# mjb3/DiscretePOMP.jl

Measured on NVIDIA B200. Metric: particle-obs steps/sec (bootstrap PF), higher is better.
Workload: dtype f32 event loop + f64 weights/scan (int32 state)

## Files before the change

### discretepomp.jl_b200/csrc/dpomp_dev.cuh

```cuda
#pragma once
#include <cuda_runtime.h>
#include <stdint.h>
#include <stdio.h>

#include "../../include/dpomp.h"

namespace dpomp {

#ifndef DPOMP_BLOCK_THREADS
#define DPOMP_BLOCK_THREADS 128
#endif
#ifndef DPOMP_ITEMS_LARGE
#define DPOMP_ITEMS_LARGE 8
#endif
#ifndef DPOMP_ITEMS_SMALL
#define DPOMP_ITEMS_SMALL 2
#endif
#ifdef DPOMP_PHASE_TIMERS
#ifndef DPOMP_PHASE_OBS
#define DPOMP_PHASE_OBS 50
#endif
static __device__ unsigned long long g_dpomp_phase[2][4096][8];
__device__ __forceinline__ unsigned long long dpomp_gtime() {
    unsigned long long t;
    asm volatile("mov.u64 %0, %%globaltimer;" : "=l"(t));
    return t;
}
#define DPOMP_STAMP(K, P)                                                                                   \
    do {                                                                                                    \
        if (threadIdx.x == 0 && a.t == DPOMP_PHASE_OBS && blockIdx.x < 4096) g_dpomp_phase[K][blockIdx.x][P] = dpomp_gtime(); \
    } while (0)
#define DPOMP_STAMP_NEXT(K, P)                                                                              \
    do {                                                                                                    \
        if (threadIdx.x == 0 && a.t == DPOMP_PHASE_OBS + 1 && blockIdx.x < 4096) g_dpomp_phase[K][blockIdx.x][P] = dpomp_gtime(); \
    } while (0)
#else
#define DPOMP_STAMP(K, P) do { } while (0)
#define DPOMP_STAMP_NEXT(K, P) do { } while (0)
#endif
#ifdef DPOMP_BOUNDS_CHECK
#define DPOMP_CHECK_IDX(i, n)                                                                                          \
    do {                                                                                                               \
        if (!((long long)(i) >= 0 && (long long)(i) < (long long)(n))) {                                               \
            printf("dpomp bounds: %s:%d: index %lld outside [0, %lld)\n", __FILE__, __LINE__, (long long)(i), (long long)(n)); \
            __trap();                                                                                                  \
        }                                                                                                              \
    } while (0)
#else
#define DPOMP_CHECK_IDX(i, n) do { } while (0)
#endif
constexpr int kBlockThreads = DPOMP_BLOCK_THREADS;
constexpr int kItemsLarge = DPOMP_ITEMS_LARGE, kItemsSmall = DPOMP_ITEMS_SMALL;

__device__ __forceinline__ void pdl_wait() {
#if __CUDA_ARCH__ >= 900
    cudaGridDependencySynchronize();
#endif
}
__device__ __forceinline__ void pdl_trigger() {
#if __CUDA_ARCH__ >= 900 && defined(DPOMP_PDL_TRIGGER)
    cudaTriggerProgrammaticLaunchCompletion();
#endif
}
template <typename... KArgs, typename... Args>
inline cudaError_t launch_pdl(void (*kern)(KArgs...), unsigned grid, unsigned block, size_t smem, cudaStream_t stream, Args... args) {
    cudaLaunchConfig_t cfg{};
    cfg.gridDim = dim3(grid);
    cfg.blockDim = dim3(block);
    cfg.dynamicSmemBytes = smem;
    cfg.stream = stream;
    cudaLaunchAttribute attr[1];
    attr[0].id = cudaLaunchAttributeProgrammaticStreamSerialization;
    attr[0].val.programmaticStreamSerializationAllowed = 1;
    cfg.attrs = attr;
    cfg.numAttrs = 1;
    return cudaLaunchKernelEx(&cfg, kern, args...);
}
constexpr int kGroupTiles = 32;
constexpr int kDeferGroups = 64;
__device__ __forceinline__ double tile_cw(double grp_off, double grp_f, double tile_o, double tile_f, double incl) {
    return __dadd_rn(grp_off, __dmul_rn(grp_f, __dadd_rn(tile_o, __dmul_rn(tile_f, incl))));
}
struct Level2 {
    double big_m, big_s;
};
template <bool CG = true>
__device__ __forceinline__ Level2 combine_level2(const double* gm_b, const double* gs_b, int ngroups, double* grp_f_out,
                                                 double* grp_off_out) {
    auto ld = [](const double* p) -> double {
        if constexpr (CG) return __ldcg(p); else return *p;
    };
    const int lane = threadIdx.x & 31;
    double big_m = -INFINITY;
    for (int i = lane; i < ngroups; i += 32) big_m = fmax(big_m, ld(gm_b + i));
#pragma unroll
    for (int d = 16; d > 0; d >>= 1) big_m = fmax(big_m, __shfl_xor_sync(0xffffffffu, big_m, d));
    double carry = 0.0;
    for (int c0 = 0; c0 < ngroups; c0 += 32) {
        const int i = c0 + lane;
        const bool have = i < ngroups;
        const double mg = have ? ld(gm_b + i) : -INFINITY;
        const double f = (mg == -INFINITY) ? 0.0 : exp(mg - big_m);
        double inc = have ? __dmul_rn(f, ld(gs_b + i)) : 0.0;
#pragma unroll
        for (int d = 1; d < 32; d <<= 1) {
            const double y = __shfl_up_sync(0xffffffffu, inc, d);
            if (lane >= d) inc = __dadd_rn(y, inc);
        }
        double prev = __shfl_up_sync(0xffffffffu, inc, 1);
        if (lane == 0) prev = 0.0;
        if (have) {
            grp_f_out[i] = f;
            grp_off_out[i] = __dadd_rn(carry, prev);
        }
        carry = __dadd_rn(carry, __shfl_sync(0xffffffffu, inc, 31));
    }
    return Level2{big_m, carry};
}
struct ChunkPerm {
    int ncf, m, q, r;
};
__host__ __device__ __forceinline__ int chunk_sigma(const ChunkPerm& p, int rr, int qq) {
    return rr * p.q + (rr < p.r ? rr : p.r) + qq;
}
__host__ __device__ __forceinline__ long long perm_pos(const ChunkPerm& p, long long i) {
    const int k = (int)(i >> 5);
    if (k >= p.ncf) return i;
    return ((long long)chunk_sigma(p, k % p.m, k / p.m) << 5) | (i & 31);
}
inline ChunkPerm make_chunk_perm(int scatter_mode, long long n, int ntiles) {
    ChunkPerm p{0, 1, 0, 0};
    if (scatter_mode != 0 && ntiles > 1) {
        p.ncf = (int)(n >> 5);
        p.m = ntiles;
        p.q = p.ncf / ntiles;
        p.r = p.ncf % ntiles;
    }
    return p;
}

constexpr uint32_t kTagSim = 0u;
constexpr uint32_t kTagResample = 1u;

struct Philox4 {
    uint32_t w0, w1, w2, w3;
};

__device__ __forceinline__ Philox4 philox4x32_10(uint32_t c0, uint32_t c1, uint32_t c2, uint32_t c3, uint32_t k0,
                                                 uint32_t k1) {
#pragma unroll
    for (int r = 0; r < 10; ++r) {
        const uint32_t hi0 = __umulhi(0xD2511F53u, c0), lo0 = 0xD2511F53u * c0;
        const uint32_t hi1 = __umulhi(0xCD9E8D57u, c2), lo1 = 0xCD9E8D57u * c2;
        const uint32_t n0 = hi1 ^ c1 ^ k0, n2 = hi0 ^ c3 ^ k1;
        c0 = n0; c1 = lo1; c2 = n2; c3 = lo0;
        k0 += 0x9E3779B9u; k1 += 0xBB67AE85u;
    }
    return Philox4{c0, c1, c2, c3};
}

__device__ __forceinline__ Philox4 stream_draw(uint64_t key, uint32_t particle, uint32_t filter, uint32_t obs,
                                               uint32_t tag, uint32_t block) {
    return philox4x32_10(particle, filter, obs, (tag << 30) | block, (uint32_t)key, (uint32_t)(key >> 32));
}

__device__ __forceinline__ uint2 philox2x32_10(uint32_t c0, uint32_t c1, uint32_t key) {
#pragma unroll
    for (int r = 0; r < 10; ++r) {
        const uint32_t hi = __umulhi(0xD256D193u, c0), lo = 0xD256D193u * c0;
        c0 = hi ^ key ^ c1;
        c1 = lo;
        key += 0x9E3779B9u;
    }
    return make_uint2(c0, c1);
}

struct SimStream {
    uint32_t k, a, b;
};
__device__ __forceinline__ SimStream sim_stream_init(uint64_t key, uint32_t filter, uint32_t obs) {
    const Philox4 p = stream_draw(key, 0u, filter, obs, kTagSim, 0u);
    return SimStream{p.w0, p.w1, p.w2};
}

__device__ __forceinline__ double u32_open_f64(uint32_t w) { return ((double)w + 0.5) * 0x1.0p-32; }
__device__ __forceinline__ float u32_wait_f32(uint32_t w) { return fmaf(__uint2float_rn(w), 0x1.0p-32f, 0x1.0p-33f); }
__device__ __forceinline__ float u32_event_f32(uint32_t w) { return __uint2float_rz(w) * 0x1.0p-32f; }
__device__ __forceinline__ double u53(uint32_t hi, uint32_t lo) {
    return (double)(((uint64_t)hi << 21) | (uint64_t)(lo >> 11)) * 0x1.0p-53;
}

template <int ITEMS, bool TAIL_SYNC = true>
__device__ __forceinline__ double tile_scan(const double (&a)[ITEMS], double (&incl)[ITEMS], double (&excl)[ITEMS],
                                            double* warp_tot) {
    const int lane = threadIdx.x & 31, warp = threadIdx.x >> 5;
    double r[ITEMS];
    r[0] = a[0];
#pragma unroll
    for (int k = 1; k < ITEMS; ++k) r[k] = __dadd_rn(r[k - 1], a[k]);
    double inc = r[ITEMS - 1];
#pragma unroll
    for (int d = 1; d < 32; d <<= 1) {
        const double y = __shfl_up_sync(0xffffffffu, inc, d);
        if (lane >= d) inc = __dadd_rn(y, inc);
    }
    double prev = __shfl_up_sync(0xffffffffu, inc, 1);
    if (lane == 0) prev = 0.0;
    if (lane == 31) warp_tot[warp] = inc;
    __syncthreads();
    double prefix = 0.0, total = 0.0;
#pragma unroll
    for (int w = 0; w < kBlockThreads / 32; ++w) {
        if (w == warp) prefix = total;
        total = __dadd_rn(total, warp_tot[w]);
    }
    const double base = __dadd_rn(prefix, prev);
#pragma unroll
    for (int k = 0; k < ITEMS; ++k) {
        incl[k] = __dadd_rn(base, r[k]);
        excl[k] = __dadd_rn(base, k > 0 ? r[k - 1] : 0.0);
    }
    if constexpr (TAIL_SYNC) __syncthreads();
    return total;
}

__device__ __forceinline__ double block_max(double v, double* warp_scratch) {
    const int lane = threadIdx.x & 31, warp = threadIdx.x >> 5;
#pragma unroll
    for (int d = 16; d > 0; d >>= 1) v = fmax(v, __shfl_xor_sync(0xffffffffu, v, d));
    if (lane == 0) warp_scratch[warp] = v;
    __syncthreads();
    double m = warp_scratch[0];
#pragma unroll
    for (int w = 1; w < kBlockThreads / 32; ++w) m = fmax(m, warp_scratch[w]);
    __syncthreads();
    return m;
}

struct ResampleCtx {
    int rs_type;
    long long n;
    double dn;
    double inv_n;
    bool pow2;
    double s;
    double inv_s;
    double r1_over_n;
    uint64_t key;
    uint32_t filter, obs;
};

__device__ __forceinline__ double div_by_n(const ResampleCtx& c, double v) {
    return c.pow2 ? v * c.inv_n : __ddiv_rn(v, c.dn);
}

template <int RS = 0>
__device__ __forceinline__ double resample_u(const ResampleCtx& c, int i ) {
    const double q = div_by_n(c, (double)(i - 1));
    double r = c.r1_over_n;
    if ((RS ? RS : c.rs_type) == DPOMP_RS_STRATIFIED) {
        const Philox4 p = stream_draw(c.key, (uint32_t)(i - 1), c.filter, c.obs, kTagResample, 1u);
        r = div_by_n(c, u53(p.w0, p.w1));
    }
    return __dmul_rn(__dadd_rn(r, q), c.s);
}

template <int RS = 0>
__device__ __forceinline__ int resample_ecount_guess(const ResampleCtx& c, double v, bool& exact) {
    const int n = (int)c.n;
    exact = true;
    if (!(c.s > 0.0)) return n;
    double g;
    if ((RS ? RS : c.rs_type) == DPOMP_RS_STRATIFIED) {
        g = floor(v * c.inv_s * c.dn);
    } else {
        const double t = (v * c.inv_s - c.r1_over_n) * c.dn;
        const double fl = floor(t);
        const double frac = t - fl;
#ifndef DPOMP_NO_ECOUNT_FAST
        if (frac > 0x1.0p-12 && frac < 1.0 - 0x1.0p-12 && t > 0.0 && t < c.dn - 1.0) return (int)fl + 1;
#endif
        g = fl + 1.0;
    }
    exact = false;
    return (int)fmin(fmax(g, 0.0), c.dn);
}
template <int RS = 0>
__device__ __forceinline__ int resample_ecount_correct(const ResampleCtx& c, double v, int e) {
    const int n = (int)c.n;
    while (e < n && resample_u<RS>(c, e + 1) <= v) ++e;
    while (e > 0 && resample_u<RS>(c, e) > v) --e;
    return e;
}
template <int RS = 0>
__device__ __forceinline__ long long resample_ecount(const ResampleCtx& c, double v) {
    bool exact;
    const int e = resample_ecount_guess<RS>(c, v, exact);
    return exact ? e : resample_ecount_correct<RS>(c, v, e);
}

__device__ __forceinline__ ResampleCtx make_resample_ctx(int rs_type, long long n, double s, uint64_t key,
                                                         uint32_t filter, uint32_t obs, double r_systematic) {
    ResampleCtx c;
    c.rs_type = rs_type;
    c.n = n;
    c.dn = (double)n;
    c.pow2 = (n & (n - 1)) == 0;
    c.inv_n = 1.0 / c.dn;
    c.s = s;
    c.inv_s = (s > 0.0) ? 1.0 / s : 0.0;
    c.key = key;
    c.filter = filter;
    c.obs = obs;
    c.r1_over_n = div_by_n(c, r_systematic);
    return c;
}

}
```

### discretepomp.jl_b200/csrc/pf_sim.cuh

```cuda
#pragma once
#include <type_traits>

#include "dpomp_dev.cuh"
#include "dpomp_internal.cuh"
#include "dpomp_models.cuh"
#include "obs_count.cuh"
#include "pf_resample.cuh"

namespace dpomp {

template <typename Real> struct Arith;
template <> struct Arith<float> {
    static __device__ __forceinline__ float mul(float a, float b) { return a * b; }
    static __device__ __forceinline__ float add(float a, float b) { return a + b; }
    static __device__ __forceinline__ float div(float a, float b) { return __fdividef(a, b); }
};
template <> struct Arith<double> {
    static __device__ __forceinline__ double mul(double a, double b) { return __dmul_rn(a, b); }
    static __device__ __forceinline__ double add(double a, double b) { return __dadd_rn(a, b); }
    static __device__ __forceinline__ double div(double a, double b) { return __ddiv_rn(a, b); }
};

#ifndef DPOMP_SIM_ILP
#define DPOMP_SIM_ILP 1
#endif
#ifndef DPOMP_SIM_PIPE
#define DPOMP_SIM_PIPE 1
#endif
#ifndef DPOMP_SIM_MINB
#define DPOMP_SIM_MINB (DPOMP_BLOCK_THREADS == 128 ? 7 : 4)
#endif
template <typename Real, int C, int E>
constexpr int sim_min_blocks() { return sizeof(Real) == 4 ? DPOMP_SIM_MINB : 1; }

template <int N>
struct alignas(4 * N) IntVec { int v[N]; };

template <typename Real, int C, int E, int MODEL>
__device__ __forceinline__ void cum_rates(const DevModel<Real, C, E>& m, const Real (&par)[E], const Real (&x)[C], Real (&cum)[E]) {
    if constexpr (MODEL != kModelGeneric) {
        using BM = Builtin<MODEL>;
#pragma unroll
        for (int e = 0; e < E; ++e) {
            Real rate = Arith<Real>::mul(par[e], x[BM::A(e)]);
            if (BM::B(e) >= 0) rate = Arith<Real>::mul(rate, x[BM::B(e) >= 0 ? BM::B(e) : 0]);
            cum[e] = (e == 0) ? rate : Arith<Real>::add(cum[e - 1], rate);
        }
    } else {
#pragma unroll
        for (int e = 0; e < E; ++e) {
            Real l1 = m.k1[e], l2 = m.k2[e];
#pragma unroll
            for (int c = 0; c < C; ++c) {
                l1 += m.f1[e][c] * x[c];
                l2 += m.f2[e][c] * x[c];
            }
            Real rate = Arith<Real>::mul(Arith<Real>::mul(par[e], l1), l2);
            if (m.any_den && m.has_den[e]) {
                Real dn = m.kd[e];
#pragma unroll
                for (int c = 0; c < C; ++c) dn += m.dn[e][c] * x[c];
                rate = (dn == (Real)0) ? (Real)0 : Arith<Real>::div(rate, dn);
            }
            cum[e] = (e == 0) ? rate : Arith<Real>::add(cum[e - 1], rate);
        }
    }
}

template <typename Real, int C, int E, int MODEL>
__device__ __forceinline__ void chosen_transition(const DevModel<Real, C, E>& m, const Real (&cum)[E], Real etc, Real (&dx)[C]) {
    if constexpr (MODEL != kModelGeneric) {
        using BM = Builtin<MODEL>;
#pragma unroll
        for (int c = 0; c < C; ++c) dx[c] = (Real)BM::T(E - 1, c);
#pragma unroll
        for (int i = E - 2; i >= 0; --i) {
            const bool hit = cum[i] > etc;
#pragma unroll
            for (int c = 0; c < C; ++c) dx[c] = hit ? (Real)BM::T(i, c) : dx[c];
        }
    } else {
#pragma unroll
        for (int c = 0; c < C; ++c) dx[c] = m.trans[E - 1][c];
#pragma unroll
        for (int i = E - 2; i >= 0; --i) {
            const bool hit = cum[i] > etc;
#pragma unroll
            for (int c = 0; c < C; ++c) dx[c] = hit ? m.trans[i][c] : dx[c];
        }
    }
}

constexpr int kModePlain = 0, kModeFused = 1, kModePersist = 2;
__device__ __forceinline__ unsigned int ld_acquire_u32(const unsigned int* p) {
    unsigned int v;
    asm volatile("ld.acquire.gpu.global.u32 %0, [%1];" : "=r"(v) : "l"(p) : "memory");
    return v;
}
constexpr int kModelCountObs = -1;
template <typename Real, int C, int E, int ITEMS, int MODEL = kModelGeneric, int MODE = kModePlain, int ILP = DPOMP_SIM_ILP>
__global__ void __launch_bounds__(kBlockThreads, sim_min_blocks<Real, C, E>())
pf_sim_weight_kernel(const __grid_constant__ DevModel<Real, C, E> m, const __grid_constant__ SimLaunch a) {
    constexpr bool COUNT = MODEL == kModelCountObs;
    constexpr int RMODEL = COUNT ? kModelGeneric : MODEL;
    constexpr int TILE = kBlockThreads * ITEMS;
    constexpr int CHUNK = 32 * ITEMS;
    constexpr bool kF32 = sizeof(Real) == 4;
    constexpr unsigned FULL = 0xffffffffu;
    constexpr bool FUSED = MODE == kModeFused, PERSIST = MODE == kModePersist;
    extern __shared__ __align__(16) unsigned char smem_raw[];
    using SState = typename std::conditional<kF32, float, int>::type;
    int* ovf_s = reinterpret_cast<int*>(smem_raw);
    SState* st_s = reinterpret_cast<SState*>(ovf_s + TILE);
    __shared__ double warp_scratch[kBlockThreads / 32];
    __shared__ unsigned warp_min_s[kBlockThreads / 32];
    __shared__ double wtab_s[kBlockThreads];
    __shared__ uint32_t stream_s[3];

    const int tid = threadIdx.x, lane = tid & 31, warp = tid >> 5;
    unsigned int logical = blockIdx.x;
    if constexpr (FUSED) {
        __shared__ unsigned int logical_s;
        if (a.work_counter) {
            if (tid == 0) logical_s = (unsigned int)(atomicAdd(a.work_counter, 1ull) - a.work_base);
            __syncthreads();
            logical = logical_s;
        }
    }
    const int tile = logical % a.ntiles;
    const int b = logical / a.ntiles;
    const long long base_n = (long long)tile * TILE;
    const uint32_t gfilter = a.filter_ids ? a.filter_ids[b] : a.filter0 + (uint32_t)b;
    const double* th = a.theta + (size_t)b * m.n_params;

    Real par[E];
#pragma unroll
    for (int e = 0; e < E; ++e) par[e] = m.par[e] >= 0 ? (Real)th[m.par[e]] : (Real)1;
    const uint32_t max_ev = (uint32_t)a.max_events;
    const int t_end = PERSIST ? a.t_last : a.t;
    int flip = 0;
    bool staged = false;
    bool wait_rows = false;
    __shared__ int warp_max_s[kBlockThreads / 32];
    __shared__ long long lohi_s[2];
    int t = a.t;
#pragma unroll 1
    do {
    const bool fresh = a.fresh && t == a.t;
    const int has_lik = PERSIST ? (a.obs_haslik[t] > 0) : a.has_lik;
    const bool do_rs = PERSIST ? (has_lik && t + 1 < a.n_obs_total) : (a.do_resample != 0);
    const bool resample_here = (FUSED || PERSIST) && do_rs;
    const double t_obs = a.obs_time[t];
    const double t_prev = fresh ? (m.t0_index > 0 ? th[m.t0_index - 1] : 0.0) : a.obs_time[t - 1];
    const double ysum = a.obs_ysum[t];
    int32_t* pop_b = ((PERSIST && (flip & 1)) ? a.pop_dst : a.pop) + (size_t)b * a.n_comp * a.n_pad;
    int32_t* pop_other = ((PERSIST && (flip & 1)) ? a.pop : a.pop_dst);
    const unsigned int gen_t = a.gen + (unsigned int)(t - a.t);

    DPOMP_STAMP(0, 0);
    DPOMP_STAMP_NEXT(0, 7);
    if (tid == 0) {
        const SimStream s0 = sim_stream_init(a.key, gfilter, (uint32_t)t);
        stream_s[0] = s0.k; stream_s[1] = s0.a; stream_s[2] = s0.b;
    }
    if constexpr (PERSIST) {
        if (wait_rows) {
            if (tid == 0) {
                const long long rem_rows = a.n - base_n;
                const unsigned int want = (unsigned int)(rem_rows < TILE ? (rem_rows > 0 ? rem_rows : 0) : TILE);
                unsigned int* cnt = a.rows_done + (size_t)b * a.ntiles + tile;
                while (ld_acquire_u32(cnt) < want) __nanosleep(40);
                *cnt = 0u;
            }
        }
        __syncthreads();
    } else {
        pdl_wait();
    }
    DPOMP_STAMP(0, 1);
    using Vec = IntVec<ITEMS>;
    {
        Vec z;
#pragma unroll
        for (int kk = 0; kk < ITEMS; ++kk) z.v[kk] = 0;
        *reinterpret_cast<Vec*>(ovf_s + tid * ITEMS) = z;
    }
    const int n_comp = (RMODEL != kModelGeneric) ? C : a.n_comp;
    if (PERSIST && staged) {
    } else if (!fresh) {
#pragma unroll
        for (int c = 0; c < C; ++c)
            if (c < n_comp)
            {
                DPOMP_CHECK_IDX(base_n + tid * ITEMS + ITEMS - 1, a.n_pad);
                const int32_t* src = pop_b + (size_t)c * a.n_pad + base_n + tid * ITEMS;
                Vec v;
                if constexpr (PERSIST) {
#pragma unroll
                    for (int kk = 0; kk < ITEMS; kk += (ITEMS % 4 == 0 ? 4 : 1)) {
                        if constexpr (ITEMS % 4 == 0) {
                            const int4 w4 = __ldcg(reinterpret_cast<const int4*>(src + kk));
                            v.v[kk] = w4.x; v.v[kk + 1] = w4.y; v.v[kk + 2] = w4.z; v.v[kk + 3] = w4.w;
                        } else {
                            v.v[kk] = __ldcg(src + kk);
                        }
                    }
                } else {
                    v = *reinterpret_cast<const Vec*>(src);
                }
#pragma unroll
                for (int kk = 0; kk < ITEMS; ++kk) st_s[c * TILE + tid * ITEMS + kk] = (SState)v.v[kk];
            }
    } else {
#pragma unroll
        for (int c = 0; c < C; ++c)
            if (c < n_comp) {
#pragma unroll
                for (int kk = 0; kk < ITEMS; ++kk) st_s[c * TILE + tid * ITEMS + kk] = (SState)m.ic[c];
            }
    }
    __syncthreads();
    DPOMP_STAMP(0, 2);
    const SimStream ss{stream_s[0], stream_s[1], stream_s[2]};

    constexpr int S = (kF32 && C <= 4 && E <= 3) ? ILP : 1;
    const int chunk0 = warp * CHUNK;
    const long long left = a.n - (base_n + chunk0);
    const int chunk_valid = left < CHUNK ? (left > 0 ? (int)left : 0) : CHUNK;
    const unsigned lt_mask = (1u << lane) - 1u;
    int next = 32 * S;
    int parked = 0;
    int q[S];
    bool active[S];
    Real x[S][C];
    Real tm[S];
    const Real tm0 = kF32 ? (Real)(t_obs - t_prev) : (Real)t_prev;
    uint32_t k[S];
    uint32_t pc[S];
    constexpr bool PIPE = DPOMP_SIM_PIPE && kF32 && S == 2;
    uint2 wn[S];
    unsigned long long ev_local = 0, ovf_local = 0;
#pragma unroll
    for (int s = 0; s < S; ++s) {
        const int slot = lane + 32 * s;
        active[s] = slot < chunk_valid;
        q[s] = chunk0 + (slot < CHUNK ? slot : lane);
        tm[s] = tm0;
        k[s] = 0;
        pc[s] = (uint32_t)(base_n + q[s]) ^ ss.a;
        if constexpr (PIPE) wn[s] = philox2x32_10(pc[s], 0u ^ ss.b, ss.k);
#pragma unroll
        for (int c = 0; c < C; ++c) x[s][c] = (c < n_comp) ? (Real)st_s[c * TILE + q[s]] : (Real)0;
    }

    while (parked < chunk_valid) {
        bool fin[S], ovf[S];
#pragma unroll
        for (int s = 0; s < S; ++s) {
            fin[s] = false;
            ovf[s] = false;
            if constexpr (kF32) {
                Real cum[E];
                cum_rates<Real, C, E, RMODEL>(m, par, x[s], cum);
                const Real rtot = cum[E - 1];
                uint2 w;
                if constexpr (PIPE) {
                    w = wn[s];
                    wn[s] = philox2x32_10(pc[s], (k[s] + 1u) ^ ss.b, ss.k);
                } else {
                    w = philox2x32_10(pc[s], k[s] ^ ss.b, ss.k);
                }
                const Real tmn = fmaf(__log2f(u32_wait_f32(w.x)), __fdividef(0.693147180559945f, rtot), tm[s]);
                const bool capped = k[s] >= max_ev;
                const bool go = (rtot > (Real)0) && !capped && (tmn >= (Real)0);
                Real dx[C];
                chosen_transition<Real, C, E, RMODEL>(m, cum, u32_event_f32(w.y) * rtot, dx);
                if (go) {
#pragma unroll
                    for (int c = 0; c < C; ++c) x[s][c] += dx[c];
                    ++k[s];
                    tm[s] = tmn;
                }
                fin[s] = active[s] && !go;
                ovf[s] = capped && (rtot > (Real)0);
            } else {
                if (active[s]) {
                    Real cum[E];
                    cum_rates<Real, C, E, RMODEL>(m, par, x[s], cum);
                    const Real rtot = cum[E - 1];
                    fin[s] = !(rtot > (Real)0);
                    if (!fin[s]) {
                        if (k[s] >= max_ev) {
                            fin[s] = true;
                            ovf[s] = true;
                        } else {
                            const uint2 w = philox2x32_10(pc[s], k[s] ^ ss.b, ss.k);
                            tm[s] = tm[s] - log(u32_open_f64(w.x)) / rtot;
                            fin[s] = tm[s] > t_obs;
                            if (!fin[s]) {
                                Real dx[C];
                                chosen_transition<Real, C, E, RMODEL>(m, cum, __dmul_rn(u32_open_f64(w.y), rtot), dx);
#pragma unroll
                                for (int c = 0; c < C; ++c) x[s][c] += dx[c];
                                ++k[s];
                            }
                        }
                    }
                }
            }
        }
#pragma unroll
        for (int s = 0; s < S; ++s) {
            const unsigned fmask = __ballot_sync(FULL, fin[s]);
            if (fmask) {
                if (fin[s]) {
                    DPOMP_CHECK_IDX(q[s], TILE);
#pragma unroll
                    for (int c = 0; c < C; ++c)
                        if (c < n_comp) st_s[c * TILE + q[s]] = (SState)x[s][c];
                    if (ovf[s]) {
                        ovf_s[q[s]] = 1;
                        ++ovf_local;
                    }
                    ev_local += k[s];
                    const int slot = next + __popc(fmask & lt_mask);
                    active[s] = slot < chunk_valid;
                    if (active[s]) {
                        q[s] = chunk0 + slot;
                        DPOMP_CHECK_IDX(q[s], TILE);
                        DPOMP_CHECK_IDX(slot, CHUNK);
                        DPOMP_CHECK_IDX(base_n + q[s], a.n);
                        pc[s] = (uint32_t)(base_n + q[s]) ^ ss.a;
#pragma unroll
                        for (int c = 0; c < C; ++c) x[s][c] = (c < n_comp) ? (Real)st_s[c * TILE + q[s]] : (Real)0;
                        tm[s] = tm0;
                        k[s] = 0;
                        if constexpr (PIPE) wn[s] = philox2x32_10(pc[s], 0u ^ ss.b, ss.k);
                    }
                }
                const int nf = __popc(fmask);
                next += nf;
                parked += nf;
            }
        }
    }
    __syncwarp();
    DPOMP_STAMP(0, 3);

    pdl_trigger();
    double av[ITEMS], incl[ITEMS], excl[ITEMS];
    auto logw_of = [&](double d) -> double {
        const double dd = __dmul_rn(d, d);
        const double quot = m.obs_tmp2_pow2 ? __dmul_rn(dd, m.obs_inv_tmp2) : __ddiv_rn(dd, m.obs_tmp2);
        return m.obs_tmp1 - quot;
    };
    constexpr unsigned kExcluded = 0xffffffffu;
    const bool int_obs = fabs(ysum) < 1073741824.0 && ysum == rint(ysum);
    double m_b;
    {
        int xs[ITEMS];
#pragma unroll
        for (int kk = 0; kk < ITEMS; ++kk) xs[kk] = 0;
#pragma unroll
        for (int c = 0; c < C; ++c)
            if (c < n_comp) {
                Vec v;
#pragma unroll
                for (int kk = 0; kk < ITEMS; ++kk) v.v[kk] = (int)st_s[c * TILE + tid * ITEMS + kk];
#pragma unroll
                for (int kk = 0; kk < ITEMS; ++kk) xs[kk] += m.xmask_i[c] * v.v[kk];
                if (!resample_here)
                    *reinterpret_cast<Vec*>(pop_b + (size_t)c * a.n_pad + base_n + tid * ITEMS) = v;
            }
        const Vec of = *reinterpret_cast<const Vec*>(ovf_s + tid * ITEMS);
        bool excluded[ITEMS];
#pragma unroll
        for (int kk = 0; kk < ITEMS; ++kk) excluded[kk] = !(base_n + tid * ITEMS + kk < a.n) || of.v[kk] != 0;

#pragma unroll
        for (int d = 16; d > 0; d >>= 1) {
            ev_local += __shfl_xor_sync(0xffffffffu, ev_local, d);
            ovf_local += __shfl_xor_sync(0xffffffffu, ovf_local, d);
        }
        if (lane == 1 && ev_local) atomicAdd(a.grp_ev + (size_t)b * a.ngroups + tile / kGroupTiles, ev_local);
        if (lane == 1 && ovf_local) atomicAdd(a.ovf_count, ovf_local);

        if constexpr (COUNT) {
            const CountObsConst cc = count_obs_const(a.cobs, th, t, ysum);
            double it[ITEMS], mloc = -INFINITY;
#pragma unroll
            for (int kk = 0; kk < ITEMS; ++kk) {
                it[kk] = excluded[kk] ? -INFINITY : count_obs_logpmf(cc, ysum, (double)xs[kk]);
                mloc = fmax(mloc, it[kk]);
            }
            if (a.record_logw) {
                double* lw_b = a.logw + (size_t)b * a.n_pad + base_n + (size_t)tid * ITEMS;
#pragma unroll
                for (int kk = 0; kk < ITEMS; ++kk) lw_b[kk] = it[kk];
            }
            m_b = block_max(mloc, warp_scratch);
            const double ref = (m_b == -INFINITY) ? 0.0 : m_b;
#pragma unroll
            for (int kk = 0; kk < ITEMS; ++kk) av[kk] = (it[kk] == -INFINITY) ? 0.0 : exp(it[kk] - ref);
        } else if (int_obs) {
            const int ys = (int)ysum;
            unsigned du[ITEMS], dloc = kExcluded;
#pragma unroll
            for (int kk = 0; kk < ITEMS; ++kk) {
                const long long df = (long long)ys - (long long)xs[kk];
                du[kk] = excluded[kk] ? kExcluded : (unsigned)(df < 0 ? -df : df);
                dloc = min(dloc, du[kk]);
            }
            dloc = __reduce_min_sync(0xffffffffu, dloc);
            if (lane == 0) warp_min_s[warp] = dloc;
            __syncthreads();
            unsigned dmin = warp_min_s[0];
#pragma unroll
            for (int w = 1; w < kBlockThreads / 32; ++w) dmin = min(dmin, warp_min_s[w]);
            if (dmin == kExcluded) {
                m_b = -INFINITY;
#pragma unroll
                for (int kk = 0; kk < ITEMS; ++kk) av[kk] = 0.0;
            } else {
                m_b = logw_of((double)dmin);
                wtab_s[tid] = exp(logw_of((double)dmin + (double)tid) - m_b);
                __syncthreads();
#pragma unroll
                for (int kk = 0; kk < ITEMS; ++kk) {
                    const unsigned off = du[kk] - dmin;
                    av[kk] = du[kk] == kExcluded ? 0.0
                           : (off < (unsigned)kBlockThreads ? wtab_s[off] : exp(logw_of((double)du[kk]) - m_b));
                    DPOMP_CHECK_IDX(du[kk] == kExcluded ? 0u : (off < (unsigned)kBlockThreads ? off : 0u), kBlockThreads);
                }
            }
            if (a.record_logw) {
                double* lw_b = a.logw + (size_t)b * a.n_pad + base_n + (size_t)tid * ITEMS;
#pragma unroll
                for (int kk = 0; kk < ITEMS; ++kk) lw_b[kk] = du[kk] == kExcluded ? -INFINITY : logw_of((double)du[kk]);
            }
        } else {
            double it[ITEMS], mloc = -INFINITY;
#pragma unroll
            for (int kk = 0; kk < ITEMS; ++kk) {
                it[kk] = excluded[kk] ? -INFINITY : logw_of(ysum - (double)xs[kk]);
                mloc = fmax(mloc, it[kk]);
            }
            if (a.record_logw) {
                double* lw_b = a.logw + (size_t)b * a.n_pad + base_n + (size_t)tid * ITEMS;
#pragma unroll
                for (int kk = 0; kk < ITEMS; ++kk) lw_b[kk] = it[kk];
            }
            m_b = block_max(mloc, warp_scratch);
            const double ref = (m_b == -INFINITY) ? 0.0 : m_b;
#pragma unroll
            for (int kk = 0; kk < ITEMS; ++kk) av[kk] = (it[kk] == -INFINITY) ? 0.0 : exp(it[kk] - ref);
        }
    }
    DPOMP_STAMP(0, 4);
    const double s_b = tile_scan<ITEMS, false>(av, incl, excl, warp_scratch);
    DPOMP_STAMP(0, 5);
    const int grp = tile / kGroupTiles;
    const int grp_tiles = min(kGroupTiles, a.ntiles - grp * kGroupTiles);
    int grp_last = 0;
    if (tid == 0) {
        a.tile_m[(size_t)b * a.ntiles + tile] = m_b;
        a.tile_s[(size_t)b * a.ntiles + tile] = s_b;
        __threadfence();
        const unsigned int ticket = atomicAdd(&a.grp_counter[(size_t)b * a.ngroups + grp], 1u);
        grp_last = (ticket == (unsigned int)(grp_tiles - 1));
    }
    if (!resample_here) {
        double* wt_b = a.wtile + (size_t)b * a.n_pad + base_n + (size_t)tid * ITEMS;
        if constexpr (ITEMS % 2 == 0) {
#pragma unroll
            for (int kk = 0; kk < ITEMS; kk += 2) *reinterpret_cast<double2*>(wt_b + kk) = make_double2(incl[kk], incl[kk + 1]);
        } else {
#pragma unroll
            for (int kk = 0; kk < ITEMS; ++kk) wt_b[kk] = incl[kk];
        }
    }
    if (tid < 32) grp_last = __shfl_sync(0xffffffffu, grp_last, 0);
    if (grp_last && tid < 32) {
    int last_group = 0;
    {
        const int i = grp * kGroupTiles + tid;
        const bool have = i < a.ntiles;
        const double mb = have ? __ldcg(a.tile_m + (size_t)b * a.ntiles + i) : -INFINITY;
        const double sb = have ? __ldcg(a.tile_s + (size_t)b * a.ntiles + i) : 0.0;
        double mg = mb;
#pragma unroll
        for (int d = 16; d > 0; d >>= 1) mg = fmax(mg, __shfl_xor_sync(0xffffffffu, mg, d));
        const double f = (mb == -INFINITY) ? 0.0 : exp(mb - mg);
        double inc = __dmul_rn(f, sb);
#pragma unroll
        for (int d = 1; d < 32; d <<= 1) {
            const double y = __shfl_up_sync(0xffffffffu, inc, d);
            if (tid >= d) inc = __dadd_rn(y, inc);
        }
        double prev = __shfl_up_sync(0xffffffffu, inc, 1);
        if (tid == 0) prev = 0.0;
        if (have) {
            a.tile_f[(size_t)b * a.ntiles + i] = f;
            a.tile_off[(size_t)b * a.ntiles + i] = prev;
        }
        if (tid == 31) {
            a.grp_m[(size_t)b * a.ngroups + grp] = mg;
            a.grp_s[(size_t)b * a.ngroups + grp] = inc;
            a.grp_counter[(size_t)b * a.ngroups + grp] = 0u;
            if (!(MODE == kModePlain && a.defer_l2)) {
                __threadfence();
                const unsigned int ticket = atomicAdd(&a.tile_counter[b], 1u);
                last_group = (ticket == (unsigned int)(a.ngroups - 1));
            }
        }
        last_group = __shfl_sync(0xffffffffu, last_group, 31);
    }
    if (last_group) {
    const Level2 l2 = combine_level2(a.grp_m + (size_t)b * a.ngroups, a.grp_s + (size_t)b * a.ngroups, a.ngroups,
                                     a.grp_f + (size_t)b * a.ngroups, a.grp_off + (size_t)b * a.ngroups);
    if (tid == 0) {
        a.filt_s[b] = l2.big_s;
        a.filt_m[b] = l2.big_m;
        if (has_lik) atomicAdd(&a.ll_acc[b], l2.big_m + log(l2.big_s / (double)a.n));
        a.tile_counter[b] = 0u;
    }
    if constexpr (FUSED) {
        __syncwarp();
        __threadfence();
        for (int g = tid; g < a.ngroups; g += 32)
            *reinterpret_cast<volatile unsigned int*>(a.gen_flags + ((size_t)b * a.ngroups + g) * 32) = a.gen;
    }
    if constexpr (PERSIST) {
        __syncwarp();
        __threadfence();
        for (int g = tid; g < a.ngroups; g += 32)
            *reinterpret_cast<volatile unsigned int*>(a.gen_flags + ((size_t)b * a.ngroups + g) * 32) = gen_t;
    }
    }
    }
    DPOMP_STAMP(0, 6);

    if constexpr (FUSED) {
        if (!do_rs) return;
        if (tid == 0) {
            const unsigned int* flag = a.gen_flags + ((size_t)b * a.ngroups + grp) * 32;
            while (ld_acquire_u32(flag) != a.gen) __nanosleep(32);
        }
        __syncthreads();
        DPOMP_STAMP(1, 1);
        const RsArgs ra{a.tile_f, a.tile_off, a.grp_f, a.grp_off, a.filt_s, nullptr, nullptr, nullptr, a.pop_dst, a.anc, a.n, a.n_pad,
                        a.ntiles, a.ngroups, a.n_comp, t, a.rs_type, a.key, a.perm};
        resample_tile<ITEMS, SState, true, 0, true, (RMODEL != kModelGeneric ? C : 0)>(ra, b, tile, gfilter, incl, st_s, TILE, ovf_s,
                                                                                      warp_max_s, lohi_s);
        DPOMP_STAMP(1, 4);
    }
    if constexpr (PERSIST) {
        if (tid == 0) {
            const unsigned int* flag = a.gen_flags + ((size_t)b * a.ngroups + grp) * 32;
            while (ld_acquire_u32(flag) != gen_t) __nanosleep(40);
        }
        __syncthreads();
        if (do_rs) {
            const RsArgs ra{a.tile_f, a.tile_off, a.grp_f, a.grp_off, a.filt_s, nullptr, nullptr, nullptr, pop_other, a.anc, a.n, a.n_pad,
                            a.ntiles, a.ngroups, a.n_comp, t, a.rs_type, a.key, a.perm};
            resample_tile<ITEMS, SState, true, 0, false>(ra, b, tile, gfilter, incl, st_s, TILE, ovf_s, warp_max_s, lohi_s);
            __threadfence();
            __syncthreads();
            const long long lo = lohi_s[0], hi = lohi_s[1];
            if (hi > lo) {
                const int d0 = (int)(lo / TILE), d1 = (int)((hi - 1) / TILE);
                for (int d = d0 + tid; d <= d1; d += kBlockThreads) {
                    const long long from = max(lo, (long long)d * TILE), to = min(hi, (long long)(d + 1) * TILE);
                    atomicAdd(a.rows_done + (size_t)b * a.ntiles + d, (unsigned int)(to - from));
                }
            }
            ++flip;
            wait_rows = true;
            staged = false;
        } else {
            wait_rows = false;
            staged = true;
        }
    }
    } while (PERSIST && ++t <= t_end);
}

template <typename Real, int C, int E>
static DevModel<Real, C, E> make_dev_model(const ModelHost& mh) {
    const dpomp_model_desc& d = mh.desc;
    DevModel<Real, C, E> m{};
    const int e_real = d.n_events;
    m.any_den = 0;
    for (int e = 0; e < E; ++e) {
        const int src = e < e_real ? e : e_real - 1;
        const bool pad = e >= e_real;
        m.par[e] = pad ? -1 : d.rate_par[src];
        m.k1[e] = pad ? (Real)0 : (Real)d.rate_k1[src];
        m.k2[e] = pad ? (Real)0 : (Real)d.rate_k2[src];
        m.kd[e] = pad ? (Real)1 : (Real)d.rate_kd[src];
        m.has_den[e] = pad ? 0 : d.rate_has_den[src];
        m.any_den |= m.has_den[e];
        for (int c = 0; c < C; ++c) {
            const bool cpad = c >= d.n_compartments;
            m.f1[e][c] = (pad || cpad) ? (Real)0 : (Real)d.rate_f1[src][c];
            m.f2[e][c] = (pad || cpad) ? (Real)0 : (Real)d.rate_f2[src][c];
            m.dn[e][c] = (pad || cpad) ? (Real)0 : (Real)d.rate_dn[src][c];
            m.trans[e][c] = cpad ? (Real)0 : (Real)d.trans[src][c];
        }
    }
    for (int c = 0; c < C; ++c) {
        const bool cpad = c >= d.n_compartments;
        m.xmask_i[c] = cpad ? 0 : (int)d.obs_xmask[c];
        m.ic[c] = cpad ? 0 : (int)d.initial_condition[c];
    }
    m.obs_tmp1 = log(1.0 / (sqrt(2.0 * 3.14159265358979323846) * d.obs_sigma));
    m.obs_tmp2 = 2.0 * d.obs_sigma * d.obs_sigma;
    {
        int ex = 0;
        m.obs_tmp2_pow2 = frexp(m.obs_tmp2, &ex) == 0.5 ? 1 : 0;
        m.obs_inv_tmp2 = 1.0 / m.obs_tmp2;
    }
    m.t0_index = d.t0_index;
    m.n_params = d.n_params;
    return m;
}

template <typename Real, int C, int E, int ITEMS, int MODEL = kModelGeneric, int ILP = DPOMP_SIM_ILP>
static int sim_inst(const ModelHost& mh, const SimLaunch& a, cudaStream_t stream, int mode) {
    constexpr int TILE = kBlockThreads * ITEMS;
    const size_t smem = (size_t)TILE * (1 + C) * sizeof(int);
    auto kern = pf_sim_weight_kernel<Real, C, E, ITEMS, MODEL, kModePlain, ILP>;
    auto kern_fused = pf_sim_weight_kernel<Real, C, E, ITEMS, MODEL, kModeFused, ILP>;
    static bool configured = false;
    if (!configured) {
        cudaFuncSetAttribute(kern, cudaFuncAttributeMaxDynamicSharedMemorySize, (int)smem);
        cudaFuncSetAttribute(kern, cudaFuncAttributePreferredSharedMemoryCarveout, cudaSharedmemCarveoutMaxShared);
        cudaFuncSetAttribute(kern_fused, cudaFuncAttributeMaxDynamicSharedMemorySize, (int)smem);
        cudaFuncSetAttribute(kern_fused, cudaFuncAttributePreferredSharedMemoryCarveout, cudaSharedmemCarveoutMaxShared);
        configured = true;
    }
    if (mode == 2) {
        int per_sm = 0, dev = 0, sms = 0;
        if (cudaOccupancyMaxActiveBlocksPerMultiprocessor(&per_sm, kern_fused, kBlockThreads, smem) != cudaSuccess) return 0;
        cudaGetDevice(&dev);
        cudaDeviceGetAttribute(&sms, cudaDevAttrMultiProcessorCount, dev);
        return per_sm * sms;
    }
    if constexpr (sizeof(Real) == 4 && MODEL > kModelGeneric) {
        auto kern_p = pf_sim_weight_kernel<Real, C, E, ITEMS, MODEL, kModePersist, ILP>;
        static bool configured_p = false;
        if (!configured_p) {
            cudaFuncSetAttribute(kern_p, cudaFuncAttributeMaxDynamicSharedMemorySize, (int)smem);
            cudaFuncSetAttribute(kern_p, cudaFuncAttributePreferredSharedMemoryCarveout, cudaSharedmemCarveoutMaxShared);
            configured_p = true;
        }
        if (mode == 4) {
            int per_sm = 0, dev = 0, sms = 0;
            if (cudaOccupancyMaxActiveBlocksPerMultiprocessor(&per_sm, kern_p, kBlockThreads, smem) != cudaSuccess) return 0;
            cudaGetDevice(&dev);
            cudaDeviceGetAttribute(&sms, cudaDevAttrMultiProcessorCount, dev);
            return per_sm * sms;
        }
        if (mode == 3) {
            const DevModel<Real, C, E> m = make_dev_model<Real, C, E>(mh);
            cudaLaunchConfig_t cfg{};
            cfg.gridDim = dim3((unsigned)(a.n_filters * a.ntiles));
            cfg.blockDim = dim3(kBlockThreads);
            cfg.dynamicSmemBytes = smem;
            cfg.stream = stream;
            cudaLaunchAttribute attr[1];
            attr[0].id = cudaLaunchAttributeCooperative;
            attr[0].val.cooperative = 1;
            cfg.attrs = attr;
            cfg.numAttrs = 1;
            return (int)cudaLaunchKernelEx(&cfg, kern_p, m, a);
        }
    }
    if (mode == 4) return 0;
    if (mode == 3) return (int)cudaErrorInvalidValue;
    const DevModel<Real, C, E> m = make_dev_model<Real, C, E>(mh);
    const unsigned grid = (unsigned)(a.n_filters * a.ntiles);
    return (int)(mode == 1 ? launch_pdl(kern_fused, grid, kBlockThreads, smem, stream, m, a)
                           : launch_pdl(kern, grid, kBlockThreads, smem, stream, m, a));
}

template <typename Real, int C, int E, int ITEMS, int MODEL>
static int sim_plain_two_per_lane(const ModelHost& mh, const SimLaunch& a, cudaStream_t stream) {
    constexpr int TILE = kBlockThreads * ITEMS;
    const size_t smem = (size_t)TILE * (1 + C) * sizeof(int);
    auto kern = pf_sim_weight_kernel<Real, C, E, ITEMS, MODEL, kModePlain, 2>;
    static bool configured = false;
    if (!configured) {
        cudaFuncSetAttribute(kern, cudaFuncAttributeMaxDynamicSharedMemorySize, (int)smem);
        cudaFuncSetAttribute(kern, cudaFuncAttributePreferredSharedMemoryCarveout, cudaSharedmemCarveoutMaxShared);
        configured = true;
    }
    const DevModel<Real, C, E> m = make_dev_model<Real, C, E>(mh);
    return (int)launch_pdl(kern, (unsigned)(a.n_filters * a.ntiles), kBlockThreads, smem, stream, m, a);
}

constexpr int kLatencyRegimeCtas = 296;
#define DPOMP_SIM_SHAPES(X) X(2, 1) X(2, 2) X(2, 3) X(3, 2) X(3, 3) X(4, 3) X(4, 6) X(8, 8)
#define DPOMP_SIM_BUILTINS(X) X(kModelSI) X(kModelSIR) X(kModelSIS) X(kModelSEI) X(kModelSEIR) X(kModelSEIS) X(kModelLOTKA)

template <typename Real>
static int sim_typed(const ModelHost& mh, int items, const SimLaunch& a, cudaStream_t stream, int mode) {
    const int c = mh.desc.n_compartments, e = mh.desc.n_events;
    const int model_id = builtin_model_id(mh.desc);
    const bool latency = sizeof(Real) == 4 && items == kItemsSmall && a.n_filters > 0 &&
                         (long long)a.n_filters * a.ntiles <= kLatencyRegimeCtas;
#define X(ID)                                                                                                             \
    if (model_id == ID) {                                                                                                 \
        if (items == kItemsSmall)                                                                                         \
            return latency ? sim_inst<Real, Builtin<ID>::C, Builtin<ID>::E, kItemsSmall, ID, 2>(mh, a, stream, mode)      \
                           : sim_inst<Real, Builtin<ID>::C, Builtin<ID>::E, kItemsSmall, ID, 1>(mh, a, stream, mode);     \
        if constexpr (sizeof(Real) == 4 && DPOMP_SIM_ILP == 1) {                                                          \
            if (mode == 0 && a.two_per_lane)                                                                              \
                return sim_plain_two_per_lane<Real, Builtin<ID>::C, Builtin<ID>::E, kItemsLarge, ID>(mh, a, stream);      \
        }                                                                                                                 \
        return sim_inst<Real, Builtin<ID>::C, Builtin<ID>::E, kItemsLarge, ID>(mh, a, stream, mode);                      \
    }
    DPOMP_SIM_BUILTINS(X)
#undef X
#define X(CC, EE)                                                                                      \
    if (c <= CC && e <= EE) {                                                                          \
        return items == kItemsSmall ? sim_inst<Real, CC, EE, kItemsSmall>(mh, a, stream, mode)         \
                                    : sim_inst<Real, CC, EE, kItemsLarge>(mh, a, stream, mode);        \
    }
    DPOMP_SIM_SHAPES(X)
#undef X
    return (mode == 2 || mode == 4) ? 0 : (int)cudaErrorInvalidValue;
}

template <typename Real>
static int sim_count_typed(const ModelHost& mh, int items, const SimLaunch& a, cudaStream_t stream, int mode) {
    if (mode == 3 || mode == 4) return mode == 4 ? 0 : (int)cudaErrorInvalidValue;
    const int c = mh.desc.n_compartments, e = mh.desc.n_events;
#define X(CC, EE)                                                                                                \
    if (c <= CC && e <= EE) {                                                                                    \
        return items == kItemsSmall ? sim_inst<Real, CC, EE, kItemsSmall, kModelCountObs>(mh, a, stream, mode) \
                                    : sim_inst<Real, CC, EE, kItemsLarge, kModelCountObs>(mh, a, stream, mode); \
    }
    DPOMP_SIM_SHAPES(X)
#undef X
    return mode == 2 ? 0 : (int)cudaErrorInvalidValue;
}

}
```

Measured before the change: 31.95 billion.

## Slim warp-refill event loop and move event/overflow tallies to ovf slots

Replaces the per-slot active flag and parked/next counters with a single head cursor compared against the chunk end. Per-particle event counts and overflow bits are packed into ovf_s, and the tallies are summed afterwards instead of kept as live 64-bit accumulators inside the loop. The waiting-time computation now uses inline PTX lg2.approx.ftz and rcp.approx.ftz in place of __log2f and __fdividef. Together these aim to shorten the loop body and lower register pressure. The risks are changed flush-to-zero behaviour for tiny rates and the tm update now being unconditional.

```diff
diff --git a/discretepomp.jl_b200/csrc/dpomp_dev.cuh b/discretepomp.jl_b200/csrc/dpomp_dev.cuh
--- a/discretepomp.jl_b200/csrc/dpomp_dev.cuh
+++ b/discretepomp.jl_b200/csrc/dpomp_dev.cuh
@@ -186,6 +186,16 @@
 __device__ __forceinline__ double u32_open_f64(uint32_t w) { return ((double)w + 0.5) * 0x1.0p-32; }
 __device__ __forceinline__ float u32_wait_f32(uint32_t w) { return fmaf(__uint2float_rn(w), 0x1.0p-32f, 0x1.0p-33f); }
 __device__ __forceinline__ float u32_event_f32(uint32_t w) { return __uint2float_rz(w) * 0x1.0p-32f; }
+__device__ __forceinline__ float lg2_ftz(float x) {
+    float y;
+    asm("lg2.approx.ftz.f32 %0, %1;" : "=f"(y) : "f"(x));
+    return y;
+}
+__device__ __forceinline__ float rcp_ftz(float x) {
+    float y;
+    asm("rcp.approx.ftz.f32 %0, %1;" : "=f"(y) : "f"(x));
+    return y;
+}
 __device__ __forceinline__ double u53(uint32_t hi, uint32_t lo) {
     return (double)(((uint64_t)hi << 21) | (uint64_t)(lo >> 11)) * 0x1.0p-53;
 }
diff --git a/discretepomp.jl_b200/csrc/pf_sim.cuh b/discretepomp.jl_b200/csrc/pf_sim.cuh
--- a/discretepomp.jl_b200/csrc/pf_sim.cuh
+++ b/discretepomp.jl_b200/csrc/pf_sim.cuh
@@ -228,10 +228,10 @@
     const long long left = a.n - (base_n + chunk0);
     const int chunk_valid = left < CHUNK ? (left > 0 ? (int)left : 0) : CHUNK;
     const unsigned lt_mask = (1u << lane) - 1u;
-    int next = 32 * S;
-    int parked = 0;
+    int head = chunk0 + 32 * S;
+    const int qend = chunk0 + chunk_valid;
+    const uint32_t g_tile = (uint32_t)base_n;
     int q[S];
-    bool active[S];
     Real x[S][C];
     Real tm[S];
     const Real tm0 = kF32 ? (Real)(t_obs - t_prev) : (Real)t_prev;
@@ -239,21 +239,21 @@
     uint32_t pc[S];
     constexpr bool PIPE = DPOMP_SIM_PIPE && kF32 && S == 2;
     uint2 wn[S];
-    unsigned long long ev_local = 0, ovf_local = 0;
 #pragma unroll
     for (int s = 0; s < S; ++s) {
         const int slot = lane + 32 * s;
-        active[s] = slot < chunk_valid;
-        q[s] = chunk0 + (slot < CHUNK ? slot : lane);
+        const int q0 = chunk0 + (slot < CHUNK ? slot : lane);
+        q[s] = chunk0 + slot;
         tm[s] = tm0;
         k[s] = 0;
-        pc[s] = (uint32_t)(base_n + q[s]) ^ ss.a;
+        pc[s] = (uint32_t)(base_n + q0) ^ ss.a;
         if constexpr (PIPE) wn[s] = philox2x32_10(pc[s], 0u ^ ss.b, ss.k);
 #pragma unroll
-        for (int c = 0; c < C; ++c) x[s][c] = (c < n_comp) ? (Real)st_s[c * TILE + q[s]] : (Real)0;
-    }
-
-    while (parked < chunk_valid) {
+        for (int c = 0; c < C; ++c) x[s][c] = (c < n_comp) ? (Real)st_s[c * TILE + q0] : (Real)0;
+    }
+
+    const int head_end = qend + 32 * S;
+    while (head < head_end) {
         bool fin[S], ovf[S];
 #pragma unroll
         for (int s = 0; s < S; ++s) {
@@ -270,7 +270,7 @@
                 } else {
                     w = philox2x32_10(pc[s], k[s] ^ ss.b, ss.k);
                 }
-                const Real tmn = fmaf(__log2f(u32_wait_f32(w.x)), __fdividef(0.693147180559945f, rtot), tm[s]);
+                const Real tmn = fmaf(lg2_ftz(u32_wait_f32(w.x)), rcp_ftz(rtot) * 0.693147180559945f, tm[s]);
                 const bool capped = k[s] >= max_ev;
                 const bool go = (rtot > (Real)0) && !capped && (tmn >= (Real)0);
                 Real dx[C];
@@ -279,12 +279,12 @@
 #pragma unroll
                     for (int c = 0; c < C; ++c) x[s][c] += dx[c];
                     ++k[s];
-                    tm[s] = tmn;
                 }
-                fin[s] = active[s] && !go;
+                tm[s] = tmn;
+                fin[s] = q[s] < qend && !go;
                 ovf[s] = capped && (rtot > (Real)0);
             } else {
-                if (active[s]) {
+                if (q[s] < qend) {
                     Real cum[E];
                     cum_rates<Real, C, E, RMODEL>(m, par, x[s], cum);
                     const Real rtot = cum[E - 1];
@@ -313,34 +313,28 @@
         for (int s = 0; s < S; ++s) {
             const unsigned fmask = __ballot_sync(FULL, fin[s]);
             if (fmask) {
+                if (ovf[s]) k[s] |= 0x80000000u;
                 if (fin[s]) {
                     DPOMP_CHECK_IDX(q[s], TILE);
 #pragma unroll
                     for (int c = 0; c < C; ++c)
                         if (c < n_comp) st_s[c * TILE + q[s]] = (SState)x[s][c];
-                    if (ovf[s]) {
-                        ovf_s[q[s]] = 1;
-                        ++ovf_local;
-                    }
-                    ev_local += k[s];
-                    const int slot = next + __popc(fmask & lt_mask);
-                    active[s] = slot < chunk_valid;
-                    if (active[s]) {
-                        q[s] = chunk0 + slot;
-                        DPOMP_CHECK_IDX(q[s], TILE);
-                        DPOMP_CHECK_IDX(slot, CHUNK);
-                        DPOMP_CHECK_IDX(base_n + q[s], a.n);
-                        pc[s] = (uint32_t)(base_n + q[s]) ^ ss.a;
-#pragma unroll
-                        for (int c = 0; c < C; ++c) x[s][c] = (c < n_comp) ? (Real)st_s[c * TILE + q[s]] : (Real)0;
-                        tm[s] = tm0;
-                        k[s] = 0;
-                        if constexpr (PIPE) wn[s] = philox2x32_10(pc[s], 0u ^ ss.b, ss.k);
-                    }
+                    ovf_s[q[s]] = (int)k[s];
                 }
-                const int nf = __popc(fmask);
-                next += nf;
-                parked += nf;
+                const int qn = head + __popc(fmask & lt_mask);
+                if (fin[s]) q[s] = qn;
+                if (fin[s] && qn < qend) {
+                    DPOMP_CHECK_IDX(qn, TILE);
+                    DPOMP_CHECK_IDX(qn - chunk0, CHUNK);
+                    DPOMP_CHECK_IDX(base_n + qn, a.n);
+                    pc[s] = (g_tile + (uint32_t)qn) ^ ss.a;
+#pragma unroll
+                    for (int c = 0; c < C; ++c) x[s][c] = (c < n_comp) ? (Real)st_s[c * TILE + qn] : (Real)0;
+                    tm[s] = tm0;
+                    k[s] = 0;
+                    if constexpr (PIPE) wn[s] = philox2x32_10(pc[s], 0u ^ ss.b, ss.k);
+                }
+                head += __popc(fmask);
             }
         }
     }
@@ -375,15 +369,21 @@
         const Vec of = *reinterpret_cast<const Vec*>(ovf_s + tid * ITEMS);
         bool excluded[ITEMS];
 #pragma unroll
-        for (int kk = 0; kk < ITEMS; ++kk) excluded[kk] = !(base_n + tid * ITEMS + kk < a.n) || of.v[kk] != 0;
-
+        for (int kk = 0; kk < ITEMS; ++kk) excluded[kk] = !(base_n + tid * ITEMS + kk < a.n) || of.v[kk] < 0;
+
+        unsigned long long ev_w = 0, ovf_w = 0;
+#pragma unroll
+        for (int kk = 0; kk < ITEMS; ++kk) {
+            ev_w += (uint32_t)of.v[kk] & 0x7fffffffu;
+            ovf_w += of.v[kk] < 0;
+        }
 #pragma unroll
         for (int d = 16; d > 0; d >>= 1) {
-            ev_local += __shfl_xor_sync(0xffffffffu, ev_local, d);
-            ovf_local += __shfl_xor_sync(0xffffffffu, ovf_local, d);
-        }
-        if (lane == 1 && ev_local) atomicAdd(a.grp_ev + (size_t)b * a.ngroups + tile / kGroupTiles, ev_local);
-        if (lane == 1 && ovf_local) atomicAdd(a.ovf_count, ovf_local);
+            ev_w += __shfl_xor_sync(0xffffffffu, ev_w, d);
+            ovf_w += __shfl_xor_sync(0xffffffffu, ovf_w, d);
+        }
+        if (lane == 1 && ev_w) atomicAdd(a.grp_ev + (size_t)b * a.ngroups + tile / kGroupTiles, ev_w);
+        if (lane == 1 && ovf_w) atomicAdd(a.ovf_count, ovf_w);
 
         if constexpr (COUNT) {
             const CountObsConst cc = count_obs_const(a.cobs, th, t, ysum);
```

Result: faster. 33.39 billion (median of 6 runs) (+4.5%).
